# thelovelab/DESeq2

Measured on AMD Instinct MI355X. Metric: genes/sec for DESeq() disp+beta+Wald fit, 50k x 500 x p=4 (throughput of steps pipelined two deep; one call at a time: one_call_at_a_time), higher is better.
Workload: dtype f64; 1 GPU; BASELINE configs[2]: 50k genes x 500 samples, ~batch+condition (p=4), Wald; 50000 non-zero genes in total, sharded over 1 GPU(s) in the contiguous ranges of R/parallel.R:10; inputs resident in HBM in R layout (int32 counts, f64 nf matrix; the fused chain reads the size factors as the m-vector the matrix was built from); genes_total=50000, genes_this_gpu=50000, samples=500, p=4, test=Wald, parallelism=gene-shard x1, chain=fused device-driven (dsq_deseq_dev), steps_overlap=step k enqueued while step k-1's results are copied and post-processed

## Files before the change

### deseq2_amd/csrc/aux.hip

```cpp
#include "dsq_internal.hpp"
#include "dsq_math.hpp"
#include "dsq_wave.hpp"

namespace dsq {

static constexpr int kAuxBatch = 4;

static inline int aux_grid_fwd(int n) {
    int blocks = (n + 3) / 4;
    int cap = device_cu_count() * 8;
    return blocks < cap ? (blocks < 1 ? 1 : blocks) : cap;
}

static constexpr int kTileS = 256;
__host__ __device__ static inline bool aux_tiled(int m, int p) { return (size_t)m * p >= 8192 && p <= 24; }

template <int P, bool USE_W, bool TILED>
__global__ void __launch_bounds__(256) prefit_kernel(PrefitKernelParams kp) {
    extern __shared__ __attribute__((aligned(16))) double tile[];
    const int lane = threadIdx.x & 63;
    const int wave = threadIdx.x >> 6;
    const int waves = blockDim.x >> 6;
    const int m = kp.m;
    double rr[P][P];
#pragma unroll
    for (int c = 0; c < P; c++)
#pragma unroll
        for (int k = 0; k < P; k++) rr[c][k] = kp.r[c + P * k];
    const int nwork = DSQ_NWORK(kp);
    for (int wbase = blockIdx.x * waves; wbase < nwork; wbase += gridDim.x * waves) {
        const int wi = wbase + wave;
        const bool active = wi < nwork;
        if (!TILED && !active) break;
        const int g = DSQ_GENE(kp, active ? wi : nwork - 1);
        const int32_t *yg = kp.y + (size_t)g * kp.ld;
        const double *nfg = kp.nf_is_vector ? kp.nf : kp.nf + (size_t)g * kp.ld;
        const double *wg = USE_W ? kp.weights + (size_t)g * kp.ld : nullptr;
        int32_t yb[kAuxBatch];
        double nb[kAuxBatch], wb[kAuxBatch];
        auto load_row = [&](int j, int b) {
            yb[b] = yg[j]; nb[b] = nfg[j];
            if constexpr (USE_W) wb[b] = wg[j];
        };
        double a2[2] = {0.0, 0.0};
        sweep_batched<kAuxBatch>(m, lane, load_row, [&](int, int b) {
            double yy = (double)yb[b];
            double cn = yy / nb[b];
            if constexpr (USE_W) cn = wb[b] * cn;
            a2[0] += cn;
            a2[1] += yy;
        });
        wave_allreduce_many(a2, lane);
        const double mean = a2[0] / (double)m;
        double av = 0.0;
        sweep_batched<kAuxBatch>(m, lane, load_row, [&](int, int b) {
            double cn = (double)yb[b] / nb[b];
            if constexpr (USE_W) cn = wb[b] * cn;
            double dlt = cn - mean;
            av += dlt * dlt;
        });
        av = wave_allreduce(av);
        double tu[2 * P];
#pragma unroll
        for (int c = 0; c < 2 * P; c++) tu[c] = 0.0;
        double ae = 0.0;
        if constexpr (TILED) {
            static_assert(kTileS == 64 * kAuxBatch, "one tile = one batch of trips");
            auto stage = [&](const double *src, int t0) {
                __syncthreads();
                const int ts = (m - t0) < kTileS ? (m - t0) : kTileS;
                for (int idx = threadIdx.x; idx < P * kTileS; idx += blockDim.x) {
                    const int c = idx / kTileS, jj = idx - c * kTileS;
                    if (jj < ts) tile[idx] = src[(size_t)c * m + t0 + jj];
                }
                __syncthreads();
            };
            for (int t0 = 0; t0 < m; t0 += kTileS) {
                stage(kp.q, t0);
                _Pragma("unroll")
                for (int b = 0; b < kAuxBatch; b++) { const int j = t0 + 64 * b + lane; if (j < m) { yb[b] = yg[j]; nb[b] = nfg[j]; } }
                _Pragma("unroll")
                for (int b = 0; b < kAuxBatch; b++) {
                    const int j = t0 + 64 * b + lane;
                    if (j < m) {
                        double yn = (double)yb[b] / nb[b];
                        double ly = dlog(yn + 0.1);
#pragma unroll
                        for (int c = 0; c < P; c++) {
                            double qv = tile[c * kTileS + 64 * b + lane];
                            tu[c] += yn * qv;
                            tu[P + c] += ly * qv;
                        }
                    }
                }
            }
            wave_allreduce_many(tu, lane);
            for (int t0 = 0; t0 < m; t0 += kTileS) {
                stage(kp.a, t0);
                _Pragma("unroll")
                for (int b = 0; b < kAuxBatch; b++) { const int j = t0 + 64 * b + lane; if (j < m) { yb[b] = yg[j]; nb[b] = nfg[j]; } }
                _Pragma("unroll")
                for (int b = 0; b < kAuxBatch; b++) {
                    const int j = t0 + 64 * b + lane;
                    if (j < m) {
                        double yn = (double)yb[b] / nb[b];
                        double mu = tu[0] * tile[64 * b + lane];
#pragma unroll
                        for (int c = 1; c < P; c++) mu = __builtin_fma(tu[c], tile[c * kTileS + 64 * b + lane], mu);
                        mu = __builtin_fmax(1.0, mu);
                        double d = yn - mu;
                        ae += (d * d - mu) / (mu * mu);
                    }
                }
            }
        } else {
        sweep_batched<kAuxBatch>(m, lane, [&](int j, int b) { yb[b] = yg[j]; nb[b] = nfg[j]; }, [&](int j, int b) {
            double yn = (double)yb[b] / nb[b];
            double ly = dlog(yn + 0.1);
#pragma unroll
            for (int c = 0; c < P; c++) {
                double qv = kp.q[(size_t)c * m + j];
                tu[c] += yn * qv;
                tu[P + c] += ly * qv;
            }
        });
        wave_allreduce_many(tu, lane);
        sweep_batched<kAuxBatch>(m, lane, [&](int j, int b) { yb[b] = yg[j]; nb[b] = nfg[j]; }, [&](int j, int b) {
            double yn = (double)yb[b] / nb[b];
            double mu = tu[0] * kp.a[j];
#pragma unroll
            for (int c = 1; c < P; c++) mu = __builtin_fma(tu[c], kp.a[(size_t)c * m + j], mu);
            mu = __builtin_fmax(1.0, mu);
            double d = yn - mu;
            ae += (d * d - mu) / (mu * mu);
        });
        }
        ae = wave_allreduce(ae);
        double b[P];
#pragma unroll
        for (int c = P - 1; c >= 0; c--) {
            double v = tu[P + c];
#pragma unroll
            for (int k = c + 1; k < P; k++) v = __builtin_fma(-rr[c][k], b[k], v);
            b[c] = v / rr[c][c];
        }
        if (lane == 0 && active) {
            kp.baseMean[g] = mean;
            kp.baseVar[g] = av / (double)(m - 1);
            kp.allZero[g] = (a2[1] == 0.0) ? 1 : 0;
            kp.roughDisp[g] = __builtin_fmax(ae / (double)(m - P), 0.0);
#pragma unroll
            for (int c = 0; c < P; c++) kp.beta_init[(size_t)g + (size_t)kp.n * c] = b[c];
        }
    }
}

template <int P, bool TILED>
__global__ void __launch_bounds__(256) linear_mu_kernel(PrefitKernelParams kp, double mu_floor, double *mu_out) {
    extern __shared__ __attribute__((aligned(16))) double tile[];
    const int lane = threadIdx.x & 63;
    const int wave = threadIdx.x >> 6;
    const int waves = blockDim.x >> 6;
    const int m = kp.m;
    const int nwork = DSQ_NWORK(kp);
    for (int wbase = blockIdx.x * waves; wbase < nwork; wbase += gridDim.x * waves) {
        const int wi = wbase + wave;
        const bool active = wi < nwork;
        if (!TILED && !active) break;
        const int g = DSQ_GENE(kp, active ? wi : nwork - 1);
        const int32_t *yg = kp.y + (size_t)g * kp.ld;
        const double *nfg = kp.nf_is_vector ? kp.nf : kp.nf + (size_t)g * kp.ld;
        double tu[P];
#pragma unroll
        for (int c = 0; c < P; c++) tu[c] = 0.0;
        if constexpr (TILED) {
            auto stage = [&](const double *src, int t0) {
                __syncthreads();
                const int ts = (m - t0) < kTileS ? (m - t0) : kTileS;
                for (int idx = threadIdx.x; idx < P * kTileS; idx += blockDim.x) {
                    const int c = idx / kTileS, jj = idx - c * kTileS;
                    if (jj < ts) tile[idx] = src[(size_t)c * m + t0 + jj];
                }
                __syncthreads();
            };
            int32_t yb[kAuxBatch];
            double nb[kAuxBatch];
            for (int t0 = 0; t0 < m; t0 += kTileS) {
                stage(kp.q, t0);
                _Pragma("unroll")
                for (int b = 0; b < kAuxBatch; b++) { const int j = t0 + 64 * b + lane; if (j < m) { yb[b] = yg[j]; nb[b] = nfg[j]; } }
                _Pragma("unroll")
                for (int b = 0; b < kAuxBatch; b++) {
                    const int j = t0 + 64 * b + lane;
                    if (j < m) {
                        double yn = (double)yb[b] / nb[b];
#pragma unroll
                        for (int c = 0; c < P; c++) tu[c] += yn * tile[c * kTileS + 64 * b + lane];
                    }
                }
            }
            wave_allreduce_many(tu, lane);
            double *mg = mu_out + (size_t)g * kp.ld;
            for (int t0 = 0; t0 < m; t0 += kTileS) {
                stage(kp.a, t0);
                _Pragma("unroll")
                for (int b = 0; b < kAuxBatch; b++) {
                    const int j = t0 + 64 * b + lane;
                    if (j < m && active) {
                        double v = tu[0] * tile[64 * b + lane];
#pragma unroll
                        for (int c = 1; c < P; c++) v = __builtin_fma(tu[c], tile[c * kTileS + 64 * b + lane], v);
                        v = v * nfg[j];
                        if (mu_floor > 0.0) v = __builtin_fmax(v, mu_floor);
                        mg[j] = v;
                    }
                }
            }
            continue;
        }
        {
// ... 284 lines not shown
    }
}

hipError_t launch_weights_prep(const double *w_raw, const double *x, int n, int m, int p, long ld, double thr, double *w_norm,
                               double *w_floor, int32_t *force_zero, int32_t *neg, hipStream_t st) {
    WeightsPrepParams kp = {n, m, p, ld, w_raw, x, thr, w_norm, w_floor, force_zero, neg};
    if (p > DSQ_P_REG) {
        const int grid = n < 256 * 8 ? n : 256 * 8;
        switch (dsq_wide_width(p)) {
#define DSQ_X(W)                                                                                                              \
        case W: {                                                                                                             \
            const size_t lds = (size_t)(3 * W * W + kRankTile * W + 2 * kRankTile) * sizeof(double);                           \
            (void)hipFuncSetAttribute(reinterpret_cast<const void *>(&weights_prep_wide_kernel<W>),                                \
                                hipFuncAttributeMaxDynamicSharedMemorySize, (int)lds);                                         \
            hipLaunchKernelGGL((weights_prep_wide_kernel<W>), dim3(grid), dim3(64), lds, st, kp);                              \
            break;                                                                                                            \
        }
        DSQ_WIDE_LIST(DSQ_X)
#undef DSQ_X
        default: return hipErrorInvalidValue;
        }
        return hipGetLastError();
    }
    hipLaunchKernelGGL(weights_prep_kernel, dim3(aux_grid_fwd(n)), dim3(256), 0, st, kp);
    return hipGetLastError();
}

__global__ void __launch_bounds__(256) xim_kernel(const double *nf, int n, int m, long ld, double *colmean_recip) {
    const int j = blockIdx.x * blockDim.x + threadIdx.x;
    if (j >= m) return;
    double s = 0.0;
    for (int g = 0; g < n; g++) s += nf[(size_t)g * ld + j];
    colmean_recip[j] = 1.0 / (s / (double)n);
}
__global__ void xim_final_kernel(const double *colmean_recip, int m, double *out) {
    if (threadIdx.x != 0 || blockIdx.x != 0) return;
    double s = 0.0;
    for (int j = 0; j < m; j++) s += colmean_recip[j];
    *out = s / (double)m;
}
__global__ void __launch_bounds__(256) xim_rows_kernel(const double *nf, const int32_t *rows, const int32_t *n_dev, int m, long ld,
                                                       double *colmean_recip) {
    const int j = blockIdx.x * blockDim.x + threadIdx.x;
    if (j >= m) return;
    const int cnt = *n_dev;
    double s = 0.0;
    for (int i = 0; i < cnt; i++) s += nf[(size_t)rows[i] * ld + j];
    colmean_recip[j] = 1.0 / (s / (double)cnt);
}
hipError_t launch_xim_rows(const double *nf, const int32_t *rows, const int32_t *n_dev, int m, long ld, double *scratch_m,
                           double *out, hipStream_t st) {
    hipLaunchKernelGGL(xim_rows_kernel, dim3((m + 255) / 256), dim3(256), 0, st, nf, rows, n_dev, m, ld, scratch_m);
    hipLaunchKernelGGL(xim_final_kernel, dim3(1), dim3(64), 0, st, (const double *)scratch_m, m, out);
    return hipGetLastError();
}
__global__ void __launch_bounds__(256) xim_flagged_kernel(const double *nf, int n, int m, long ld, const int32_t *want_a,
                                                          const int32_t *want_b, double *colmean_recip) {
    const int j = blockIdx.x * blockDim.x + threadIdx.x;
    if (j >= m) return;
    double s = 0.0;
    int cnt = 0;
    for (int g = 0; g < n; g++)
        if (want_a[g] != 0 && want_b[g] == 0) { s += nf[(size_t)g * ld + j]; cnt++; }
    colmean_recip[j] = 1.0 / (s / (double)cnt);
}
hipError_t launch_xim_flagged(const double *nf, int n, int m, long ld, const int32_t *want_a, const int32_t *want_b, double *scratch_m,
                              double *out, hipStream_t st) {
    hipLaunchKernelGGL(xim_flagged_kernel, dim3((m + 255) / 256), dim3(256), 0, st, nf, n, m, ld, want_a, want_b, scratch_m);
    hipLaunchKernelGGL(xim_final_kernel, dim3(1), dim3(64), 0, st, (const double *)scratch_m, m, out);
    return hipGetLastError();
}
hipError_t launch_xim(const double *nf, int n, int m, long ld, double *scratch_m, double *out, hipStream_t st) {
    hipLaunchKernelGGL(xim_kernel, dim3((m + 255) / 256), dim3(256), 0, st, nf, n, m, ld, scratch_m);
    hipLaunchKernelGGL(xim_final_kernel, dim3(1), dim3(64), 0, st, (const double *)scratch_m, m, out);
    return hipGetLastError();
}

static inline int aux_grid(int n) {
    int blocks = (n + 3) / 4;
    int cap = device_cu_count() * 8;
    return blocks < cap ? (blocks < 1 ? 1 : blocks) : cap;
}

template <int P>
static hipError_t launch_prefit_p(const PrefitKernelParams &kp, hipStream_t st) {
    if constexpr (P <= 24) {
        if (aux_tiled(kp.m, P)) {
            const size_t lds = (size_t)P * kTileS * sizeof(double);
            if (kp.useWeights) hipLaunchKernelGGL((prefit_kernel<P, true, true>), dim3(aux_grid(kp.n)), dim3(256), lds, st, kp);
            else hipLaunchKernelGGL((prefit_kernel<P, false, true>), dim3(aux_grid(kp.n)), dim3(256), lds, st, kp);
            return hipGetLastError();
        }
    }
    if (kp.useWeights) hipLaunchKernelGGL((prefit_kernel<P, true, false>), dim3(aux_grid(kp.n)), dim3(256), 0, st, kp);
    else hipLaunchKernelGGL((prefit_kernel<P, false, false>), dim3(aux_grid(kp.n)), dim3(256), 0, st, kp);
    return hipGetLastError();
}

hipError_t launch_prefit(const PrefitKernelParams &kp, hipStream_t st, bool *ok) {
    *ok = true;
    switch (kp.p) {
#define DSQ_X(W) case W: return launch_prefit_p<W>(kp, st);
    DSQ_P_EACH(DSQ_X)
#undef DSQ_X
    default: *ok = false; return hipSuccess;
    }
}

template <int P>
static hipError_t launch_linear_mu_p(const PrefitKernelParams &kp, double mu_floor, double *mu, hipStream_t st) {
    if constexpr (P <= 24) {
        if (aux_tiled(kp.m, P)) {
            hipLaunchKernelGGL((linear_mu_kernel<P, true>), dim3(aux_grid(kp.n)), dim3(256), (size_t)P * kTileS * sizeof(double), st, kp, mu_floor, mu);
            return hipGetLastError();
        }
    }
    hipLaunchKernelGGL((linear_mu_kernel<P, false>), dim3(aux_grid(kp.n)), dim3(256), 0, st, kp, mu_floor, mu);
    return hipGetLastError();
}

hipError_t launch_linear_mu(const PrefitKernelParams &kp, double mu_floor, double *mu, hipStream_t st, bool *ok) {
    *ok = true;
    switch (kp.p) {
#define DSQ_X(W) case W: return launch_linear_mu_p<W>(kp, mu_floor, mu, st);
    DSQ_P_EACH(DSQ_X)
#undef DSQ_X
    default: *ok = false; return hipSuccess;
    }
}

hipError_t launch_intercept_fit(const InterceptKernelParams &kp, hipStream_t st) {
    if (kp.useWeights) hipLaunchKernelGGL((intercept_fit_kernel<true>), dim3(aux_grid(kp.n)), dim3(256), 0, st, kp);
    else hipLaunchKernelGGL((intercept_fit_kernel<false>), dim3(aux_grid(kp.n)), dim3(256), 0, st, kp);
    return hipGetLastError();
}

hipError_t launch_loglike(const LogLikeKernelParams &kp, hipStream_t st) {
    if (kp.useWeights) hipLaunchKernelGGL((loglike_kernel<true>), dim3(aux_grid(kp.n)), dim3(256), 0, st, kp);
    else hipLaunchKernelGGL((loglike_kernel<false>), dim3(aux_grid(kp.n)), dim3(256), 0, st, kp);
    return hipGetLastError();
}
hipError_t launch_loglike_side(const LogLikeKernelParams &kp, hipStream_t st) {
    int grid = aux_grid(kp.n);
    const int cap = device_cu_count() * 6;
    if (grid > cap) grid = cap;
    if (kp.useWeights) hipLaunchKernelGGL((loglike_kernel<true>), dim3(grid), dim3(256), 0, st, kp);
    else hipLaunchKernelGGL((loglike_kernel<false>), dim3(grid), dim3(256), 0, st, kp);
    return hipGetLastError();
}

}
```

### deseq2_amd/csrc/pipeline.hip

```cpp
#include "capi.hpp"
#include "dsq_math.hpp"
#include "dsq_wave.hpp"

#include <algorithm>
#include <cstdio>
#include <cstdlib>
#include <cstring>
#include <vector>

namespace dsq {

DSQ_DEV double np_min(double a, double b) { return (a != a || b != b) ? a + b : (a < b ? a : b); }
DSQ_DEV double np_max(double a, double b) { return (a != a || b != b) ? a + b : (a > b ? a : b); }

struct Rows {
    const int32_t *rows;
    const int32_t *n_dev;
    int n;
};
DSQ_DEV int rows_count(const Rows &r) { return r.n_dev ? *r.n_dev : r.n; }
DSQ_DEV int rows_gene(const Rows &r, int i) { return r.rows ? r.rows[i] : i; }

__global__ void __launch_bounds__(1024) compact_kernel(int mode, int n, int32_t *allZero, const int32_t *force_zero,
                                                       const double *mean_in, const double *disp_in, double thresh,
                                                       int32_t *rows_out, double *mean_out, double *disp_out,
                                                       int32_t *count_out) {
    constexpr int NT = 4;
    __shared__ int wcnt[NT][16];
    __shared__ int base_s;
    const int t = threadIdx.x, lane = t & 63, wave = t >> 6;
    if (t == 0) base_s = 0;
    __syncthreads();
    for (int i0 = 0; i0 < n; i0 += NT * 1024) {
        bool keep[NT];
        double mv[NT], dv[NT];
#pragma unroll
        for (int q = 0; q < NT; q++) {
            const int i = i0 + q * 1024 + t;
            keep[q] = false; mv[q] = 0.0; dv[q] = 0.0;
            if (i < n) {
                if (mode == 0) {
                    int z = allZero[i] | (force_zero ? force_zero[i] : 0);
                    if (force_zero) allZero[i] = z ? 1 : 0;
                    keep[q] = !z;
                } else {
                    dv[q] = disp_in[i]; mv[q] = mean_in[i];
                    keep[q] = dv[q] > thresh;
                }
            }
        }
        unsigned long long mask[NT];
#pragma unroll
        for (int q = 0; q < NT; q++) {
            mask[q] = __ballot(keep[q]);
            if (lane == 0) wcnt[q][wave] = __popcll(mask[q]);
        }
        __syncthreads();
        int off = base_s;
#pragma unroll
        for (int q = 0; q < NT; q++) {
            int mine = off;
            for (int w = 0; w < 16; w++) { const int c = wcnt[q][w]; if (w < wave) mine += c; off += c; }
            mine += __popcll(mask[q] & ((1ull << lane) - 1ull));
            if (keep[q]) {
                const int i = i0 + q * 1024 + t;
                if (mode == 0) rows_out[mine] = i;
                else { mean_out[mine] = mv[q]; disp_out[mine] = dv[q]; }
            }
        }
        __syncthreads();
        if (t == 0) base_s = off;
        __syncthreads();
    }
    if (t == 0) *count_out = base_s;
}

constexpr int kLptBins = 128;
enum { LPT_NONE = 0, LPT_MEAN_UP = 1, LPT_MEAN_DOWN = 2, LPT_ITER = 3, LPT_ITER_F64 = 4, LPT_ITER_MEAN = 5, LPT_DIST = 6 };
struct LptKey {
    int kind;
    const int32_t *ki;
    const double *kd, *kd2;
};
DSQ_DEV int lpt_bin(const LptKey &k, int g) {
    double kd;
    if (k.kind == LPT_MEAN_UP || k.kind == LPT_MEAN_DOWN) {
        kd = 127.0 - 8.656170245333781 * dlog(1.0 + k.kd[g]);
        if (kd < 0.0) kd = 0.0;
        if (k.kind == LPT_MEAN_DOWN) kd = 127.0 - kd;
    } else if (k.kind == LPT_ITER) {
        kd = (double)k.ki[g];
    } else if (k.kind == LPT_ITER_MEAN) {
        kd = 0.25 * (double)k.ki[g] * (1.4426950408889634 * dlog(2.0 + k.kd[g]));
    } else if (k.kind == LPT_DIST) {
        kd = 16.0 * __builtin_fabs(k.kd[g] - k.kd2[g]);
    } else {
        kd = k.kd[g];
    }
    if (!(kd >= 0.0)) kd = 127.0;
    return kd > 127.0 ? 127 : (int)kd;
}
DSQ_DEV void lpt_block_hist(int bin, int *bins) {
    __shared__ int h[kLptBins];
    for (int k = threadIdx.x; k < kLptBins; k += blockDim.x) h[k] = 0;
    __syncthreads();
    if (bin >= 0) atomicAdd(&h[bin], 1);
    __syncthreads();
    for (int k = threadIdx.x; k < kLptBins; k += blockDim.x)
        if (h[k]) atomicAdd(&bins[k], h[k]);
}

struct RuleParams {
    Rows rw;
    int n;
    int p;
    double minDisp, maxDisp, xim, outlierSD;
    const double *xim_dev;
    int maxit, betaMaxit;
    const double *baseMean, *baseVar, *roughDisp;
    double *alpha_init, *la0;
    const double *la_out, *initial_lp, *last_lp;
    const int32_t *iter;
    const double *la_grid;
    double *dge;
    int32_t *dispGeneIter;
    int32_t *grid_flag, *grid_rows, *grid_count;
    const double *scalars;
    double *dispFit, *log_dfit, *la_init, *dispMAP, *dispersion;
    const double *dispFit_in;
    int32_t *dispIter, *dispOutlier;
    const double *beta_nat, *beta_var, *beta_iter, *logLike;
    double *beta, *betaSE, *stat, *pvalue, *betaIter_out;
    int32_t *betaConv, *optim_flag, *optim_count;
    int32_t *optim_rows;
    int wald;
    const double *beta_init;
    double *opt_start;
    const int32_t *opt_conv;
    LptKey lpt;
    int *lpt_bins;
};

__global__ void alpha_init_kernel(RuleParams q) {
    const int i = blockIdx.x * blockDim.x + threadIdx.x;
    const bool on = i < rows_count(q.rw);
    const int g = on ? rows_gene(q.rw, i) : 0;
    if (on) {
        const double bm = q.baseMean[g], bv = q.baseVar[g];
        const double xim = q.xim_dev ? *q.xim_dev : q.xim;
        const double mom = (bv - xim * bm) / (bm * bm);
        double a = np_min(q.roughDisp[g], mom);
        a = np_min(np_max(q.minDisp, a), q.maxDisp);
        q.alpha_init[g] = a;
        q.la0[g] = dlog(a);
    }
    if (q.lpt.kind != LPT_NONE) lpt_block_hist(on ? lpt_bin(q.lpt, g) : -1, q.lpt_bins);
}
// ... 1011 lines not shown
    if (a->phases & DSQ_PH_GENE_EST) {
        struct Fill { char *p; size_t bytes; uint32_t val; };
        std::vector<Fill> fills;
        auto fill = [&](void *p_, size_t bytes, uint32_t val) { if (p_ && bytes) fills.push_back({(char *)p_, bytes, val}); };
        fill(o->status, DSQ_ST_COUNT * sizeof(int32_t), 0u);
        for (OutF64 v : kNaVectors) fill(o->*v, (size_t)n * sizeof(double), 0xFFFFFFFFu);
        for (OutF64 v : kNaMatrices) fill(o->*v, (size_t)n * (a->betaPrior ? a->p_prior : p) * sizeof(double), 0xFFFFFFFFu);
        if (a->betaPrior) fill(o->mle_beta, (size_t)n * p * sizeof(double), 0xFFFFFFFFu);
        for (OutI32 v : kNaInts) fill(o->*v, (size_t)n * sizeof(int32_t), 0xFFFFFFFFu);
        for (OutI32 v : kZeroInts) fill(o->*v, (size_t)n * sizeof(int32_t), 0u);
        fill(P.grid_flag, (size_t)n * sizeof(int32_t), 0u);
        std::sort(fills.begin(), fills.end(), [](const Fill &x, const Fill &y) { return x.p < y.p; });
        for (const Fill &fl : fills) f.add(fl.p, fl.bytes, fl.val);
    }
    if (a->phases & DSQ_PH_TREND) {
        f.add(o->scalars + DSQ_SC_FIT_USED, sizeof(double), 0u);
        int rc;
        if (!a->dispFit_in && a->fitType != DSQ_FIT_MEAN) {
            if ((rc = capi_ws_get(DSQ_WS_PIPE_META, trend_fit_workspace_bytes() + 64, &P.trend_ws))) return rc;
            f.add(P.trend_ws, (trend_fit_workspace_bytes() + 3) / 4 * 4, 0u);
        }
        const size_t sel_bytes = prior_var_workspace_bytes(trend_count(P));
        if (sel_bytes) {
            if ((rc = capi_ws_get(DSQ_WS_PIPE_SEL, sel_bytes + 64, &P.sel_ws))) return rc;
            f.add(P.sel_ws, (sel_bytes + 3) / 4 * 4, 0u);
        }
    }
    if (f.full) return capi_fail(DSQ_ERR_DEVICE, "dsq_deseq_dev: more than %d init segments", kInitSegMax);
    size_t words = 0;
    for (int sgi = 0; sgi < ip.nseg; sgi++) words += ip.seg[sgi].words;
    unsigned blocks = (unsigned)((words + 256 * 8 - 1) / (256 * 8));
    if (blocks < 1) blocks = 1;
    if (blocks > 2048) blocks = 2048;
    hipLaunchKernelGGL(chain_init_kernel, dim3(blocks), dim3(256), 0, P.st, ip);
    DSQ_HIP(hipGetLastError());
    return DSQ_OK;
}

static int prepare_designs(Pipe &P) {
    const DsqDeseqArgs *a = P.a;
    const int n = P.n, m = P.m, p = P.p, pk = P.pk;
    hipStream_t st = P.st;
    int rc;
    P.x_k = a->x;
    if (pk > p) {
        if ((rc = capi_pad_design(DSQ_WS_PIPE_PADX, a->x, m, p, pk, st, &P.x_k))) return rc;
        P.padmask = dsq_low_bits(pk) & ~dsq_low_bits(p);
        DSQ_HIP(hipMemsetAsync(P.beta_init + (size_t)n * p, 0, (size_t)n * (pk - p) * sizeof(double), st));
        DSQ_HIP(hipMemsetAsync(P.opt_start + (size_t)n * p, 0, (size_t)n * (pk - p) * sizeof(double), st));
    }
    P.red_x_k = a->x_red; P.red_pk = a->x_red ? kern_width(a->p_red) : 0; P.red_lam = a->x_red ? P.lam_prior : P.lam;
    if (P.red_pk > a->p_red) {
        if ((rc = capi_pad_design(DSQ_WS_PIPE_PADXR, a->x_red, m, a->p_red, P.red_pk, st, &P.red_x_k))) return rc;
        DSQ_HIP(hipMemsetAsync(P.red_binit + (size_t)n * a->p_red, 0, (size_t)n * (P.red_pk - a->p_red) * sizeof(double), st));
    }
    P.pri_x_k = a->x_prior; P.pri_pk = P.pkp;
    if (a->betaPrior && P.pkp > a->p_prior)
        if ((rc = capi_pad_design(DSQ_WS_PIPE_PADXR, a->x_prior, m, a->p_prior, P.pkp, st, &P.pri_x_k))) return rc;
    if (a->cell_of && a->ncell > 0)
        P.ncell = capi_upload_cells(a->cell_of, m, DSQ_WS_PIPE_CELLS, st, &P.cell_perm, &P.cell_start);
    if (a->x_red || a->betaPrior) {
        if (a->x_red && a->cell_of_red && a->ncell_red > 0)
            P.red_ncell = capi_upload_cells(a->cell_of_red, m, DSQ_WS_PIPE_CELLS_RED, st, &P.red_cell_perm, &P.red_cell_start);
        void *b;
        if ((rc = capi_ws_get(DSQ_WS_PIPE_RED_MU, (size_t)n * P.ld * sizeof(double), &b))) return rc;
        P.red_mu = (double *)b;
    }
    return DSQ_OK;
}

static int xim_scratch(const Pipe &P, double **out) {
    void *b;
    const int rc = capi_ws_get(DSQ_WS_PIPE_XIM_SCRATCH, ((size_t)P.m + 8) * sizeof(double), &b);
    *out = (double *)b;
    return rc;
}

static int phase_gene_est(Pipe &P, const Rows &nz) {
    const DsqDeseqArgs *a = P.a;
    const DsqDeseqOut *o = P.o;
    const Rows all = {nullptr, nullptr, P.n};
    int rc = launch_prefit_rows(P, all, a->y);
    if (rc) return rc;
    hipLaunchKernelGGL(compact_kernel, dim3(1), dim3(1024), 0, P.st, 0, P.n, o->allZero, a->force_zero,
                       (const double *)nullptr, (const double *)nullptr, 0.0, P.rows_nz, (double *)nullptr,
                       (double *)nullptr, P.counters + CNT_NZ);
    if (!a->nf_is_vector) {
        double *b;
        if ((rc = xim_scratch(P, &b))) return rc;
        DSQ_HIP(launch_xim_rows(a->nf, P.rows_nz, P.counters + CNT_NZ, P.m, P.ld, b, P.xim_dev, P.st));
    }
    return gene_est(P, nz, a->y, o->mu_hat, CNT_GRID1, CNT_OPT1, o->optim_geneest);
}

static int phase_trend(Pipe &P) {
    const DsqDeseqArgs *a = P.a;
    const DsqDeseqOut *o = P.o;
    hipStream_t st = P.st;
    const double *tm = a->trend_mean ? a->trend_mean : o->baseMean;
    const double *td = a->trend_mean ? a->trend_disp : o->dispGeneEst;
    const int nt = trend_count(P);
    if (!(a->phases & DSQ_PH_GENE_EST)) DSQ_HIP(hipMemsetAsync(P.counters + CNT_TREND, 0, sizeof(int32_t), st));
    hipLaunchKernelGGL(compact_kernel, dim3(1), dim3(1024), 0, st, 1, nt, (int32_t *)nullptr, (const int32_t *)nullptr,
                       tm, td, 100.0 * a->minDisp, (int32_t *)nullptr, P.trend_mean_c, P.trend_disp_c,
                       P.counters + CNT_TREND);
    capi_prof_begin("trend_fit", nt, st);
    hipError_t e = hipSuccess;
    if (a->dispFit_in) {
        e = launch_trend_given(o->scalars, o->status, st);
    } else {
        if (a->fitType != DSQ_FIT_MEAN)
            e = launch_trend_fit_dev_zeroed(P.trend_mean_c, P.trend_disp_c, P.counters + CNT_TREND, o->scalars + DSQ_SC_COEF0,
                                            o->status + DSQ_ST_TREND_STATUS, P.trend_ws, st);
        if (e == hipSuccess && a->fitType != DSQ_FIT_PARAMETRIC)
            e = launch_trend_mean(td, nt, a->minDisp, (int)a->fitType, o->scalars, o->status, st);
    }
    capi_prof_end(st);
    DSQ_HIP(e);
    capi_prof_begin("prior_var", nt, st);
    const double *fin = a->dispFit_in ? (a->trend_mean ? a->trend_fit_in : a->dispFit_in) : (const double *)nullptr;
    e = launch_prior_var(tm, td, nt, a->minDisp, a->expVarLogDisp, (P.m > P.p) ? 1 : 0, P.resbuf, o->scalars, o->status, fin,
                         a->dispPriorVar_in, P.sel_ws, st);
    capi_prof_end(st);
    DSQ_HIP(e);
    return DSQ_OK;
}

static int phase_map_test(Pipe &P, const Rows &nz, bool *counters_zeroed) {
    const DsqDeseqArgs *a = P.a;
    const DsqDeseqOut *o = P.o;
    if (!(a->phases & DSQ_PH_GENE_EST)) {
        DSQ_HIP(hipMemsetAsync(P.counters + CNT_GRID2, 0, sizeof(int32_t), P.st));
        DSQ_HIP(hipMemsetAsync(P.counters + CNT_OPT2, 0, sizeof(int32_t), P.st));
        DSQ_HIP(hipMemsetAsync(P.counters + CNT_OPT3, 0, sizeof(int32_t), P.st));
    }
    int rc = map_est(P, nz, a->y, o->mu_hat, CNT_GRID2);
    if (rc) return rc;
    if ((rc = test_fit(P, nz, a->y, o->mu, o->H, CNT_OPT2))) return rc;
    const bool z = *counters_zeroed = (a->phases & (DSQ_PH_OUTLIERS | DSQ_PH_OUTLIERS_DETECT)) && !((a->phases & DSQ_PH_PRIOR) && a->betaPrior);
    hipLaunchKernelGGL(na_assay_rows_kernel, ew_grid(P.n), dim3(256), 0, P.st, P.n, P.m, P.ld, (const int32_t *)o->allZero, o->mu, o->H,
                       z ? P.counters + CNT_REP : (int32_t *)nullptr, z ? (int)(CNT_N - CNT_REP) : 0);
    return DSQ_OK;
}

static int phase_prior(Pipe &P, const Rows &nz) {
    DSQ_HIP(hipMemsetAsync(P.counters + CNT_OPT2, 0, sizeof(int32_t), P.st));
    return prior_fit(P, nz, P.a->y, CNT_OPT2);
}

static CooksKernelParams cooks_params(const Pipe &P, const OutlierMeta &M, const Rows &rw) {
    const DsqDeseqArgs *a = P.a;
    const DsqDeseqOut *o = P.o;
    CooksKernelParams ck;
    memset(&ck, 0, sizeof ck);
    ck.n = P.n; ck.m = P.m; ck.p = P.p; ck.ld = P.ld; ck.y = a->y; ck.nf = a->nf; ck.nf_is_vector = a->nf_is_vector;
    ck.mu = o->mu; ck.H = o->H; ck.perm = M.dperm; ck.cell_start = M.dstart; ck.in3 = M.din3; ck.ncell = a->ncell; ck.any3 = M.any3;
    int cap = 2; while (cap < (M.any3 ? M.maxcell : P.m)) cap <<= 1;
    ck.sortcap = cap;
    ck.cooks = o->cooks; ck.maxCooks = o->maxCooks; ck.robustDisp = P.robustDisp;
    ck.rows = rw.rows; ck.n_dev = rw.n_dev;
    return ck;
}
static ReplaceKernelParams replace_params(const Pipe &P, const OutlierMeta &M, const Rows &rw) {
    const DsqDeseqArgs *a = P.a;
    const DsqDeseqOut *o = P.o;
    ReplaceKernelParams rk;
    memset(&rk, 0, sizeof rk);
    rk.n = P.n; rk.m = P.m; rk.ld = P.ld; rk.y = a->y; rk.nf = a->nf; rk.nf_is_vector = a->nf_is_vector;
    rk.cooks = o->cooks; rk.cutoff = a->cooksCutoff; rk.trim = a->trim; rk.replaceable = M.drepl;
    int cap2 = 2; while (cap2 < P.m) cap2 <<= 1;
    rk.sortcap = cap2;
    rk.newCounts = o->replaceCounts; rk.replace = o->replace;
    rk.rows = rw.rows; rk.n_dev = rw.n_dev;
    return rk;
}
static int launch_cooks_rows(Pipe &P, const CooksKernelParams &ck, hipStream_t st) {
    bool ok = true;
    capi_prof_begin("cooks_distance", P.n, st);
    DSQ_HIP(launch_cooks(ck, st, &ok));
    capi_prof_end(st);
    if (!ok) return capi_fail(DSQ_ERR_UNSUPPORTED, "m=%d samples: a gene row plus its sort buffer exceeds the 160 KiB LDS", P.m);
    return DSQ_OK;
}
static int launch_replace_rows(Pipe &P, const ReplaceKernelParams &rk, hipStream_t st) {
    bool ok = true;
    capi_prof_begin("replace_outliers", P.n, st);
    DSQ_HIP(launch_replace(rk, st, &ok));
    capi_prof_end(st);
// ... 139 lines not shown
```

Before: 5.770 million genes/s.

## Fuse prefit sweeps with row caching and parallelize stream compaction across blocks

The prefit kernel now computes mean, log-projection, variance and rough-dispersion moments in two sweeps instead of four. Normalized counts from the first sweep are kept in registers (m<=512) or LDS (m<=1024) so the second sweep does not reload counts and size factors. Separately, the single-block compaction kernel is replaced by a two-kernel count/scan/write scheme spread over many blocks, which removes a serial bottleneck over 50k genes. The cost is more template instances, more LDS or registers per block, one extra kernel launch per compaction, and tile counts that reuse the resbuf scratch buffer.

```diff
diff --git a/deseq2_amd/csrc/aux.hip b/deseq2_amd/csrc/aux.hip
--- a/deseq2_amd/csrc/aux.hip
+++ b/deseq2_amd/csrc/aux.hip
@@ -15,7 +15,16 @@
 static constexpr int kTileS = 256;
 __host__ __device__ static inline bool aux_tiled(int m, int p) { return (size_t)m * p >= 8192 && p <= 24; }
 
-template <int P, bool USE_W, bool TILED>
+enum { KEEP_NONE = 0, KEEP_REGS = 1, KEEP_LDS = 2 };
+static constexpr int kKeepRegs = 8;
+static constexpr int kKeepLdsM = 1024;
+static inline int aux_keep(int m, int p, bool tiled) {
+    if (m <= 64 * kKeepRegs) return KEEP_REGS;
+    const size_t lds = ((tiled ? (size_t)p * kTileS : 0) + (size_t)4 * m) * sizeof(double);
+    return (m <= kKeepLdsM && lds <= 65536) ? KEEP_LDS : KEEP_NONE;
+}
+
+template <int P, bool USE_W, bool TILED, int KEEP>
 __global__ void __launch_bounds__(256) prefit_kernel(PrefitKernelParams kp) {
     extern __shared__ __attribute__((aligned(16))) double tile[];
     const int lane = threadIdx.x & 63;
@@ -42,7 +51,113 @@
             yb[b] = yg[j]; nb[b] = nfg[j];
             if constexpr (USE_W) wb[b] = wg[j];
         };
+        static_assert(kTileS == 64 * kAuxBatch, "one tile = one batch of trips");
+        auto stage = [&](const double *src, int t0) {
+            __syncthreads();
+            const int ts = (m - t0) < kTileS ? (m - t0) : kTileS;
+            for (int idx = threadIdx.x; idx < P * kTileS; idx += blockDim.x) {
+                const int c = idx / kTileS, jj = idx - c * kTileS;
+                if (jj < ts) tile[idx] = src[(size_t)c * m + t0 + jj];
+            }
+            __syncthreads();
+        };
+        (void)stage;
         double a2[2] = {0.0, 0.0};
+        double mean, av = 0.0, ae = 0.0;
+        double tu[2 * P];
+#pragma unroll
+        for (int c = 0; c < 2 * P; c++) tu[c] = 0.0;
+        if constexpr (KEEP != KEEP_NONE) {
+            constexpr int kGroups = kKeepRegs / kAuxBatch;
+            double yk[KEEP == KEEP_REGS ? kKeepRegs : 1];
+            double *ys = tile + (TILED ? P * kTileS : 0) + (size_t)wave * m;
+            auto keep_put = [&](int gi, int b, int j, double v) {
+                if constexpr (KEEP == KEEP_REGS) {
+                    _Pragma("unroll")
+                    for (int s = 0; s < kGroups; s++) yk[kAuxBatch * s + b] = (s == gi) ? v : yk[kAuxBatch * s + b];
+                } else ys[j] = v;
+            };
+            auto keep_get = [&](int gi, int b, int j) {
+                if constexpr (KEEP == KEEP_REGS) {
+                    double v = yk[b];
+                    _Pragma("unroll")
+                    for (int s = 1; s < kGroups; s++) v = (s == gi) ? yk[kAuxBatch * s + b] : v;
+                    return v;
+                } else return ys[j];
+            };
+            if constexpr (KEEP == KEEP_REGS) {
+                _Pragma("unroll")
+                for (int s = 0; s < kKeepRegs; s++) yk[s] = 0.0;
+            }
+            auto for_groups = [&](auto &&body) {
+                _Pragma("nounroll")
+                for (int gi = 0; gi * kTileS < m; gi++) body(gi);
+            };
+            for_groups([&](int gi) {
+                const int t0 = gi * kTileS;
+                if constexpr (TILED) stage(kp.q, t0);
+                _Pragma("unroll")
+                for (int b = 0; b < kAuxBatch; b++) { const int j = t0 + 64 * b + lane; if (j < m) load_row(j, b); }
+                _Pragma("unroll")
+                for (int b = 0; b < kAuxBatch; b++) {
+                    const int j = t0 + 64 * b + lane;
+                    if (j < m) {
+                        double yy = (double)yb[b];
+                        double yn = yy / nb[b];
+                        keep_put(gi, b, j, yn);
+                        double cn = yn;
+                        if constexpr (USE_W) cn = wb[b] * cn;
+                        a2[0] += cn;
+                        a2[1] += yy;
+                        double ly = dlog(yn + 0.1);
+#pragma unroll
+                        for (int c = 0; c < P; c++) {
+                            double qv;
+                            if constexpr (TILED) qv = tile[c * kTileS + 64 * b + lane];
+                            else qv = kp.q[(size_t)c * m + j];
+                            tu[c] += yn * qv;
+                            tu[P + c] += ly * qv;
+                        }
+                    }
+                }
+            });
+            wave_allreduce_many(a2, lane);
+            wave_allreduce_many(tu, lane);
+            mean = a2[0] / (double)m;
+            for_groups([&](int gi) {
+                const int t0 = gi * kTileS;
+                if constexpr (TILED) stage(kp.a, t0);
+                if constexpr (USE_W) {
+                    _Pragma("unroll")
+                    for (int b = 0; b < kAuxBatch; b++) { const int j = t0 + 64 * b + lane; if (j < m) wb[b] = wg[j]; }
+                }
+                _Pragma("unroll")
+                for (int b = 0; b < kAuxBatch; b++) {
+                    const int j = t0 + 64 * b + lane;
+                    if (j < m) {
+                        const double yn = keep_get(gi, b, j);
+                        double cn = yn;
+                        if constexpr (USE_W) cn = wb[b] * cn;
+                        double dlt = cn - mean;
+                        av += dlt * dlt;
+                        double mu;
+                        if constexpr (TILED) {
+                            mu = tu[0] * tile[64 * b + lane];
+#pragma unroll
+                            for (int c = 1; c < P; c++) mu = __builtin_fma(tu[c], tile[c * kTileS + 64 * b + lane], mu);
+                        } else {
+                            mu = tu[0] * kp.a[j];
+#pragma unroll
+                            for (int c = 1; c < P; c++) mu = __builtin_fma(tu[c], kp.a[(size_t)c * m + j], mu);
+                        }
+                        mu = __builtin_fmax(1.0, mu);
+                        double d = yn - mu;
+                        ae += (d * d - mu) / (mu * mu);
+                    }
+                }
+            });
+            wave_allreduce_pair(av, ae, lane);
+        } else {
         sweep_batched<kAuxBatch>(m, lane, load_row, [&](int, int b) {
             double yy = (double)yb[b];
             double cn = yy / nb[b];
@@ -51,8 +166,7 @@
             a2[1] += yy;
         });
         wave_allreduce_many(a2, lane);
-        const double mean = a2[0] / (double)m;
-        double av = 0.0;
+        mean = a2[0] / (double)m;
         sweep_batched<kAuxBatch>(m, lane, load_row, [&](int, int b) {
             double cn = (double)yb[b] / nb[b];
             if constexpr (USE_W) cn = wb[b] * cn;
@@ -60,21 +174,7 @@
             av += dlt * dlt;
         });
         av = wave_allreduce(av);
-        double tu[2 * P];
-#pragma unroll
-        for (int c = 0; c < 2 * P; c++) tu[c] = 0.0;
-        double ae = 0.0;
         if constexpr (TILED) {
-            static_assert(kTileS == 64 * kAuxBatch, "one tile = one batch of trips");
-            auto stage = [&](const double *src, int t0) {
-                __syncthreads();
-                const int ts = (m - t0) < kTileS ? (m - t0) : kTileS;
-                for (int idx = threadIdx.x; idx < P * kTileS; idx += blockDim.x) {
-                    const int c = idx / kTileS, jj = idx - c * kTileS;
-                    if (jj < ts) tile[idx] = src[(size_t)c * m + t0 + jj];
-                }
-                __syncthreads();
-            };
             for (int t0 = 0; t0 < m; t0 += kTileS) {
                 stage(kp.q, t0);
                 _Pragma("unroll")
@@ -136,6 +236,7 @@
         });
         }
         ae = wave_allreduce(ae);
+        }
         double b[P];
 #pragma unroll
         for (int c = P - 1; c >= 0; c--) {
@@ -586,19 +687,32 @@
     return blocks < cap ? (blocks < 1 ? 1 : blocks) : cap;
 }
 
+template <int P, bool TILED, int KEEP>
+static hipError_t launch_prefit_pk(const PrefitKernelParams &kp, hipStream_t st) {
+    const size_t lds = ((TILED ? (size_t)P * kTileS : 0) + (KEEP == KEEP_LDS ? (size_t)4 * kp.m : 0)) * sizeof(double);
+    if (kp.useWeights) hipLaunchKernelGGL((prefit_kernel<P, true, TILED, KEEP>), dim3(aux_grid(kp.n)), dim3(256), lds, st, kp);
+    else hipLaunchKernelGGL((prefit_kernel<P, false, TILED, KEEP>), dim3(aux_grid(kp.n)), dim3(256), lds, st, kp);
+    return hipGetLastError();
+}
+template <int P, bool TILED>
+static hipError_t launch_prefit_pt(const PrefitKernelParams &kp, hipStream_t st) {
+    if constexpr (P <= DSQ_P_REG) {
+        switch (aux_keep(kp.m, P, TILED)) {
+        case KEEP_REGS:
+            if constexpr (!TILED) return launch_prefit_pk<P, TILED, KEEP_REGS>(kp, st);
+            break;
+        case KEEP_LDS: return launch_prefit_pk<P, TILED, KEEP_LDS>(kp, st);
+        default: break;
+        }
+    }
+    return launch_prefit_pk<P, TILED, KEEP_NONE>(kp, st);
+}
 template <int P>
 static hipError_t launch_prefit_p(const PrefitKernelParams &kp, hipStream_t st) {
     if constexpr (P <= 24) {
-        if (aux_tiled(kp.m, P)) {
-            const size_t lds = (size_t)P * kTileS * sizeof(double);
-            if (kp.useWeights) hipLaunchKernelGGL((prefit_kernel<P, true, true>), dim3(aux_grid(kp.n)), dim3(256), lds, st, kp);
-            else hipLaunchKernelGGL((prefit_kernel<P, false, true>), dim3(aux_grid(kp.n)), dim3(256), lds, st, kp);
-            return hipGetLastError();
-        }
-    }
-    if (kp.useWeights) hipLaunchKernelGGL((prefit_kernel<P, true, false>), dim3(aux_grid(kp.n)), dim3(256), 0, st, kp);
-    else hipLaunchKernelGGL((prefit_kernel<P, false, false>), dim3(aux_grid(kp.n)), dim3(256), 0, st, kp);
-    return hipGetLastError();
+        if (aux_tiled(kp.m, P)) return launch_prefit_pt<P, true>(kp, st);
+    }
+    return launch_prefit_pt<P, false>(kp, st);
 }
 
 hipError_t launch_prefit(const PrefitKernelParams &kp, hipStream_t st, bool *ok) {
diff --git a/deseq2_amd/csrc/pipeline.hip b/deseq2_amd/csrc/pipeline.hip
--- a/deseq2_amd/csrc/pipeline.hip
+++ b/deseq2_amd/csrc/pipeline.hip
@@ -21,58 +21,65 @@
 DSQ_DEV int rows_count(const Rows &r) { return r.n_dev ? *r.n_dev : r.n; }
 DSQ_DEV int rows_gene(const Rows &r, int i) { return r.rows ? r.rows[i] : i; }
 
-__global__ void __launch_bounds__(1024) compact_kernel(int mode, int n, int32_t *allZero, const int32_t *force_zero,
-                                                       const double *mean_in, const double *disp_in, double thresh,
-                                                       int32_t *rows_out, double *mean_out, double *disp_out,
-                                                       int32_t *count_out) {
-    constexpr int NT = 4;
-    __shared__ int wcnt[NT][16];
+constexpr int kCompactTile = 1024;
+struct CompactParams {
+    int mode, n;
+    int32_t *allZero;
+    const int32_t *force_zero;
+    const double *mean_in, *disp_in;
+    double thresh;
+    int32_t *tile_cnt;
+    int32_t *rows_out;
+    double *mean_out, *disp_out;
+    int32_t *count_out;
+};
+DSQ_DEV bool compact_keep(const CompactParams &c, int i) {
+    if (i >= c.n) return false;
+    if (c.mode == 0) return !(c.allZero[i] | (c.force_zero ? c.force_zero[i] : 0));
+    return c.disp_in[i] > c.thresh;
+}
+__global__ void __launch_bounds__(kCompactTile) compact_count_kernel(CompactParams c) {
+    __shared__ int wcnt[kCompactTile / 64];
+    const int t = threadIdx.x, lane = t & 63, wave = t >> 6;
+    const unsigned long long mask = __ballot(compact_keep(c, blockIdx.x * kCompactTile + t));
+    if (lane == 0) wcnt[wave] = __popcll(mask);
+    __syncthreads();
+    if (t == 0) {
+        int s = 0;
+        for (int w = 0; w < kCompactTile / 64; w++) s += wcnt[w];
+        c.tile_cnt[blockIdx.x] = s;
+    }
+}
+__global__ void __launch_bounds__(kCompactTile) compact_write_kernel(CompactParams c) {
+    __shared__ int wcnt[kCompactTile / 64];
     __shared__ int base_s;
     const int t = threadIdx.x, lane = t & 63, wave = t >> 6;
-    if (t == 0) base_s = 0;
+    const int i = blockIdx.x * kCompactTile + t;
+    const bool keep = compact_keep(c, i);
+    if (c.mode == 0 && c.force_zero && i < c.n) c.allZero[i] = keep ? 0 : 1;
+    const unsigned long long mask = __ballot(keep);
+    if (lane == 0) wcnt[wave] = __popcll(mask);
+    if (wave == 0) {
+        int s = 0;
+        for (int k = lane; k < (int)blockIdx.x; k += 64) s += c.tile_cnt[k];
+        for (int o = 32; o > 0; o >>= 1) s += __shfl_xor(s, o, 64);
+        if (lane == 0) base_s = s;
+    }
     __syncthreads();
-    for (int i0 = 0; i0 < n; i0 += NT * 1024) {
-        bool keep[NT];
-        double mv[NT], dv[NT];
-#pragma unroll
-        for (int q = 0; q < NT; q++) {
-            const int i = i0 + q * 1024 + t;
-            keep[q] = false; mv[q] = 0.0; dv[q] = 0.0;
-            if (i < n) {
-                if (mode == 0) {
-                    int z = allZero[i] | (force_zero ? force_zero[i] : 0);
-                    if (force_zero) allZero[i] = z ? 1 : 0;
-                    keep[q] = !z;
-                } else {
-                    dv[q] = disp_in[i]; mv[q] = mean_in[i];
-                    keep[q] = dv[q] > thresh;
-                }
-            }
-        }
-        unsigned long long mask[NT];
-#pragma unroll
-        for (int q = 0; q < NT; q++) {
-            mask[q] = __ballot(keep[q]);
-            if (lane == 0) wcnt[q][wave] = __popcll(mask[q]);
-        }
-        __syncthreads();
-        int off = base_s;
-#pragma unroll
-        for (int q = 0; q < NT; q++) {
-            int mine = off;
-            for (int w = 0; w < 16; w++) { const int c = wcnt[q][w]; if (w < wave) mine += c; off += c; }
-            mine += __popcll(mask[q] & ((1ull << lane) - 1ull));
-            if (keep[q]) {
-                const int i = i0 + q * 1024 + t;
-                if (mode == 0) rows_out[mine] = i;
-                else { mean_out[mine] = mv[q]; disp_out[mine] = dv[q]; }
-            }
-        }
-        __syncthreads();
-        if (t == 0) base_s = off;
-        __syncthreads();
-    }
-    if (t == 0) *count_out = base_s;
+    int mine = base_s, total = base_s;
+    for (int w = 0; w < kCompactTile / 64; w++) { const int k = wcnt[w]; if (w < wave) mine += k; total += k; }
+    mine += __popcll(mask & ((1ull << lane) - 1ull));
+    if (keep) {
+        if (c.mode == 0) c.rows_out[mine] = i;
+        else { c.mean_out[mine] = c.mean_in[i]; c.disp_out[mine] = c.disp_in[i]; }
+    }
+    if (t == 0 && blockIdx.x == gridDim.x - 1) *c.count_out = total;
+}
+static hipError_t launch_compact(CompactParams c, hipStream_t st) {
+    const int tiles = c.n > 0 ? (c.n + kCompactTile - 1) / kCompactTile : 1;
+    hipLaunchKernelGGL(compact_count_kernel, dim3(tiles), dim3(kCompactTile), 0, st, c);
+    hipLaunchKernelGGL(compact_write_kernel, dim3(tiles), dim3(kCompactTile), 0, st, c);
+    return hipGetLastError();
 }
 
 constexpr int kLptBins = 128;
@@ -1250,9 +1257,11 @@
     const Rows all = {nullptr, nullptr, P.n};
     int rc = launch_prefit_rows(P, all, a->y);
     if (rc) return rc;
-    hipLaunchKernelGGL(compact_kernel, dim3(1), dim3(1024), 0, P.st, 0, P.n, o->allZero, a->force_zero,
-                       (const double *)nullptr, (const double *)nullptr, 0.0, P.rows_nz, (double *)nullptr,
-                       (double *)nullptr, P.counters + CNT_NZ);
+    CompactParams c;
+    memset(&c, 0, sizeof c);
+    c.mode = 0; c.n = P.n; c.allZero = o->allZero; c.force_zero = a->force_zero;
+    c.tile_cnt = (int32_t *)P.resbuf; c.rows_out = P.rows_nz; c.count_out = P.counters + CNT_NZ;
+    DSQ_HIP(launch_compact(c, P.st));
     if (!a->nf_is_vector) {
         double *b;
         if ((rc = xim_scratch(P, &b))) return rc;
@@ -1269,9 +1278,11 @@
     const double *td = a->trend_mean ? a->trend_disp : o->dispGeneEst;
     const int nt = trend_count(P);
     if (!(a->phases & DSQ_PH_GENE_EST)) DSQ_HIP(hipMemsetAsync(P.counters + CNT_TREND, 0, sizeof(int32_t), st));
-    hipLaunchKernelGGL(compact_kernel, dim3(1), dim3(1024), 0, st, 1, nt, (int32_t *)nullptr, (const int32_t *)nullptr,
-                       tm, td, 100.0 * a->minDisp, (int32_t *)nullptr, P.trend_mean_c, P.trend_disp_c,
-                       P.counters + CNT_TREND);
+    CompactParams c;
+    memset(&c, 0, sizeof c);
+    c.mode = 1; c.n = nt; c.mean_in = tm; c.disp_in = td; c.thresh = 100.0 * a->minDisp;
+    c.tile_cnt = (int32_t *)P.resbuf; c.mean_out = P.trend_mean_c; c.disp_out = P.trend_disp_c; c.count_out = P.counters + CNT_TREND;
+    DSQ_HIP(launch_compact(c, st));
     capi_prof_begin("trend_fit", nt, st);
     hipError_t e = hipSuccess;
     if (a->dispFit_in) {
```

After: 5.840 million genes/s, median of 6. +1.2%, better.
